# ashys2012/MDC-Net-Multimodal-Defect-Captioning-Network-For-Surface-Steel-Defects

Measured on NVIDIA B200. Metric: images/sec end-to-end encode+greedy decode, higher is better.
Workload: dtype bf16

## Files before the change

mdc-net-multimodal-defect-captioning-network-for-surface-steel-defects_b200/csrc/attention_umma.cu:

```cuda
#include "common.cuh"
#include <cuda.h>
#include <stdlib.h>

namespace {

constexpr int HD = 64;
constexpr int QROWS = 256;
constexpr int N_SOFTMAX_WARPS = 16;
constexpr int THREADS = 64 + N_SOFTMAX_WARPS * 32;

struct SmemLayout {
  int q_bytes, kv_bytes, buf_bytes;
};

__global__ void __launch_bounds__(THREADS, 1)
attn_umma_kernel(const __grid_constant__ CUtensorMap map_q, const __grid_constant__ CUtensorMap map_kv, bf16* __restrict__ out, int64_t ldo,
                 int n_items, int S, int H, int NK, float scale_log2e, long long* dbg) {
#ifdef MDC_DEVTOOLS
#define STAMP(i) do { if (dbg && blockIdx.x == 0 && n == 0) dbg[i] = clock64(); } while (0)
#else
#define STAMP(i) do { } while (0)
#endif
  extern __shared__ uint8_t smem_raw[];
  uint8_t* smem = (uint8_t*)(((uintptr_t)smem_raw + 1023) & ~(uintptr_t)1023);
  const int q_bytes = QROWS * 128, kv_bytes = NK * 128, buf_bytes = q_bytes + 2 * kv_bytes;
  uint64_t* bars = (uint64_t*)(smem + 2 * buf_bytes);
  uint64_t* full = bars; uint64_t* sfree = bars + 2; uint64_t* s_ready = bars + 4; uint64_t* p_ready = bars + 6; uint64_t* o_ready = bars + 8;
  uint64_t* t_free = bars + 10;
  uint32_t* tmem_ptr_smem = (uint32_t*)(bars + 12);
  float* xch = (float*)(bars + 16);
  const int warp = threadIdx.x >> 5, lane = threadIdx.x & 31;
  const int tiles = S > 128 ? 2 : 1;

  if (threadIdx.x == 0) {
    for (int i = 0; i < 2; ++i) {
      mbar_init(smem_u32(&full[i]), 1); mbar_init(smem_u32(&sfree[i]), 1); mbar_init(smem_u32(&s_ready[i]), 1);
      mbar_init(smem_u32(&p_ready[i]), N_SOFTMAX_WARPS * 32); mbar_init(smem_u32(&o_ready[i]), 1); mbar_init(smem_u32(&t_free[i]), N_SOFTMAX_WARPS * 32);
    }
    fence_mbarrier_init();
    prefetch_tmap(&map_q);
    prefetch_tmap(&map_kv);
  }
  if (warp == 0) {
    tmem_alloc<1>(smem_u32(tmem_ptr_smem), 512);
    tmem_relinquish<1>();
  }
  tc_fence_before();
  __syncthreads();
  tc_fence_after();
  const uint32_t tmem_base = *tmem_ptr_smem;
  const int D = H * HD;

  if (warp == 1) {
    if (lane == 0) {
      int n = 0;
      for (int item = blockIdx.x; item < n_items; item += gridDim.x, ++n) {
        const int buf = n & 1, strip = item / H, head = item % H;
        mbar_wait(smem_u32(&sfree[buf]), ((n >> 1) & 1) ^ 1);
        const uint32_t fb = smem_u32(&full[buf]);
        const uint32_t base = smem_u32(smem + buf * buf_bytes);
        STAMP(0);
        mbar_expect_tx(fb, (uint32_t)(3 * kv_bytes));
        tma_load_2d(&map_kv, fb, base, head * HD, strip * S);
        tma_load_2d(&map_kv, fb, base + q_bytes, D + head * HD, strip * S);
        tma_load_2d(&map_kv, fb, base + q_bytes + kv_bytes, 2 * D + head * HD, strip * S);
      }
    }
  } else if (warp == 0) {
    if (lane == 0) {
      const uint32_t idesc_qk = make_idesc(128, NK), idesc_pv = make_idesc(128, HD, false, true);
      int n = 0;
      for (int item = blockIdx.x; item < n_items; item += gridDim.x, ++n) {
        const int buf = n & 1;
        const uint32_t base = smem_u32(smem + buf * buf_bytes);
        mbar_wait(smem_u32(&full[buf]), (n >> 1) & 1);
        STAMP(1);
        tc_fence_after();
        const uint64_t kdesc = make_sw128_desc(base + q_bytes);
        for (int t = 0; t < tiles; ++t) {
          mbar_wait(smem_u32(&t_free[t]), (n & 1) ^ 1);
          tc_fence_after();
          const uint64_t qdesc = make_sw128_desc(base + t * 128 * 128);
#pragma unroll
          for (int k = 0; k < HD / 16; ++k) umma_ss(tmem_base + t * 256, qdesc + 2 * k, kdesc + 2 * k, idesc_qk, k != 0);
          umma_commit(smem_u32(&s_ready[t]));
          STAMP(2 + t);
        }
        const uint64_t vdesc = make_sw128_desc(base + q_bytes + kv_bytes);
        for (int t = 0; t < tiles; ++t) {
          mbar_wait(smem_u32(&p_ready[t]), n & 1);
          STAMP(4 + t);
          tc_fence_after();
          for (int k = 0; k < NK / 16; ++k)
            umma_ts(tmem_base + t * 256 + 128, tmem_base + t * 256 + 8 * k, vdesc + (uint64_t)(128 * k), idesc_pv, k != 0);
          umma_commit(smem_u32(&o_ready[t]));
          STAMP(6 + t);
        }
        umma_commit(smem_u32(&sfree[buf]));
      }
    }
  } else {
    const int sw = warp - 2, part = sw >> 2, row = 32 * (warp & 3) + lane;
    const int qc = NK / 4;
    const int nch = qc / 4;
    const uint32_t lane_addr = (uint32_t)(32 * (warp & 3)) << 16;
    int n = 0;
    for (int item = blockIdx.x; item < n_items; item += gridDim.x, ++n) {
      const int strip = item / H, head = item % H;
      float rsum[2] = {0.f, 0.f};
      for (int t = 0; t < tiles; ++t) {
        mbar_wait(smem_u32(&s_ready[t]), n & 1);
        if (threadIdx.x == 64) STAMP(10 + 8 * t);
        tc_fence_after();
        const uint32_t trow = tmem_base + lane_addr + t * 256;
        const bool live = __any_sync(0xffffffffu, t * 128 + row < S);
        float s[64];
        if (live) {
          uint32_t* sr = reinterpret_cast<uint32_t*>(s);
          const uint32_t tcol = trow + part * qc;
          if (nch >= 8) {
            tmem_ld32(tcol, sr);
            if (nch == 16) tmem_ld32(tcol + 32, sr + 32);
            else if (nch >= 12) {
              tmem_ld16(tcol + 32, sr + 32);
#pragma unroll
              for (int c = 12; c < 15; ++c) if (c < nch) tmem_ld4(tcol + 4 * c, sr + 4 * c);
            } else {
#pragma unroll
              for (int c = 8; c < 11; ++c) if (c < nch) tmem_ld4(tcol + 4 * c, sr + 4 * c);
            }
          } else if (nch >= 4) {
            tmem_ld16(tcol, sr);
#pragma unroll
            for (int c = 4; c < 7; ++c) if (c < nch) tmem_ld4(tcol + 4 * c, sr + 4 * c);
          } else {
#pragma unroll
            for (int c = 0; c < 3; ++c) if (c < nch) tmem_ld4(tcol + 4 * c, sr + 4 * c);
          }
          tmem_ld_wait();
        }
        if (threadIdx.x == 64) STAMP(11 + 8 * t);
        const int nvalid = min(max(S - part * qc, 0), qc);
        float m4[4] = {-INFINITY, -INFINITY, -INFINITY, -INFINITY};
        if (live) {
#pragma unroll
          for (int c = 0; c < 16; ++c)
            if (c < nch) {
              if (4 * c + 4 <= nvalid) {
#pragma unroll
                for (int j = 0; j < 4; ++j) m4[j] = fmaxf(m4[j], s[4 * c + j]);
              } else {
#pragma unroll
                for (int j = 0; j < 4; ++j) {
                  if (4 * c + j >= nvalid) s[4 * c + j] = -INFINITY;
                  m4[j] = fmaxf(m4[j], s[4 * c + j]);
                }
              }
            }
        }
        float mx = fmaxf(fmaxf(m4[0], m4[1]), fmaxf(m4[2], m4[3]));
        xch[part * 128 + row] = mx;
        bar_sync<128>(1 + (warp & 3));
        if (threadIdx.x == 64) STAMP(12 + 8 * t);
        mx = fmaxf(fmaxf(xch[row], xch[128 + row]), fmaxf(xch[256 + row], xch[384 + row]));
        const float nms = -mx * scale_log2e;
        float s4[4] = {0.f, 0.f, 0.f, 0.f};
        if (live) {
#pragma unroll
          for (int c = 0; c < 16; ++c)
            if (c < nch) {
              float p[4];
#pragma unroll
              for (int j = 0; j < 4; ++j) { p[j] = ex2_approx(fmaf(s[4 * c + j], scale_log2e, nms)); s4[j] += p[j]; }
              tmem_st2(trow + (part * qc) / 2 + 2 * c, pack_bf16x2(p[0], p[1]), pack_bf16x2(p[2], p[3]));
            }
        }
        const float sum = (s4[0] + s4[1]) + (s4[2] + s4[3]);
        rsum[t] = sum;
        xch[512 + t * 512 + part * 128 + row] = sum;
        if (threadIdx.x == 64) STAMP(13 + 8 * t);
        tmem_st_wait();
        if (threadIdx.x == 64) STAMP(14 + 8 * t);
        tc_fence_before();
        mbar_arrive(smem_u32(&p_ready[t]));
        bar_sync<128>(1 + (warp & 3));
      }
      for (int t = 0; t < tiles; ++t) {
        mbar_wait(smem_u32(&o_ready[t]), n & 1);
        if (threadIdx.x == 64) STAMP(26 + 2 * t);
        tc_fence_after();
        const uint32_t trow = tmem_base + lane_addr + t * 256 + 128;
        uint32_t o[16];
        tmem_ld16(trow + part * 16, o);
        tmem_ld_wait();
        tc_fence_before();
        mbar_arrive(smem_u32(&t_free[t]));
        const float* sx = xch + 512 + t * 512 + row;
        const float inv = 1.0f / ((sx[0] + sx[128]) + (sx[256] + sx[384]));
        const int q = t * 128 + row;
        if (q < S) {
          bf16* dst = out + ((int64_t)strip * S + q) * ldo + head * HD + part * 16;
#pragma unroll
          for (int j = 0; j < 16; j += 8) {
            uint4 v;
            v.x = pack_bf16x2(__uint_as_float(o[j]) * inv, __uint_as_float(o[j + 1]) * inv);
            v.y = pack_bf16x2(__uint_as_float(o[j + 2]) * inv, __uint_as_float(o[j + 3]) * inv);
            v.z = pack_bf16x2(__uint_as_float(o[j + 4]) * inv, __uint_as_float(o[j + 5]) * inv);
            v.w = pack_bf16x2(__uint_as_float(o[j + 6]) * inv, __uint_as_float(o[j + 7]) * inv);
            *reinterpret_cast<uint4*>(dst + j) = v;
          }
        }
      }
      if (threadIdx.x == 64) STAMP(30);
      bar_sync<128>(1 + (warp & 3));
    }
  }
  tc_fence_before();
  __syncthreads();
  if (warp == 0) {
    tc_fence_after();
    tmem_dealloc<1>(tmem_base, 512);
  }
}

}

int attn_umma_supported(int strip_len, int head_dim, int64_t ld, int64_t ldo) {
  return head_dim == HD && strip_len >= 16 && strip_len <= 256 && ld % 8 == 0 && ldo % 8 == 0;
}

int attn_umma_launch(mdc_ctx* ctx, const void* qkv, int64_t ld, void* out, int64_t ldo, int n_strips, int strip_len, int heads, float scale,
                     cudaStream_t s) {
  MDC_CHECK_ARG(((uintptr_t)qkv & 15) == 0 && ((uintptr_t)out & 15) == 0);
  const int S = strip_len, NK = ((S + 15) / 16) * 16;
  const int64_t rows = (int64_t)n_strips * S;
  CUtensorMap mq, mkv;
  MDC_TRY(mdc_make_tmap_2d(ctx, qkv, rows, 3 * heads * HD, ld, HD, NK, 3, &mkv));
  mq = mkv;
  const int buf_bytes = QROWS * 128 + 2 * NK * 128;
  const size_t smem = 2 * (size_t)buf_bytes + 1024 + 128 + 3 * 512 * 4;
  MDC_ENSURE_SMEM(attn_umma_kernel, smem);
  const int n_items = n_strips * heads;
  const int grid = n_items < ctx->sm_count ? n_items : ctx->sm_count;
  long long* dbg = nullptr;
#ifdef MDC_DEVTOOLS
  if (const char* e = getenv("MDC_ATTN_TRACE_PTR")) dbg = (long long*)strtoull(e, nullptr, 0);
#endif
  attn_umma_kernel<<<grid, THREADS, smem, s>>>(mq, mkv, (bf16*)out, ldo, n_items, S, heads, NK, scale * LOG2E, dbg);
  MDC_LAUNCH_CHECK(ctx);
  return 0;
}
```

mdc-net-multimodal-defect-captioning-network-for-surface-steel-defects_b200/csrc/ptx.cuh:

```cuda
#pragma once
#include <cuda.h>
#include <cuda_bf16.h>
#include <cuda_fp16.h>
#include <stdint.h>

__device__ __forceinline__ uint32_t smem_u32(const void* p) { return (uint32_t)__cvta_generic_to_shared(p); }
__device__ __forceinline__ uint32_t mapa(uint32_t addr, uint32_t rank) {
  uint32_t r; asm volatile("mapa.shared::cluster.u32 %0, %1, %2;" : "=r"(r) : "r"(addr), "r"(rank)); return r;
}
__device__ __forceinline__ uint32_t cluster_rank() { uint32_t r; asm volatile("mov.u32 %0, %%cluster_ctarank;" : "=r"(r)); return r; }
__device__ __forceinline__ void cluster_sync() {
  asm volatile("barrier.cluster.arrive.release.aligned;\n\tbarrier.cluster.wait.acquire.aligned;" ::: "memory");
}
__device__ __forceinline__ bool elect_one() {
  uint32_t pred;
  asm volatile("{\n\t.reg .pred P;\n\telect.sync _|P, 0xffffffff;\n\tselp.u32 %0, 1, 0, P;\n\t}\n" : "=r"(pred));
  return pred != 0;
}
__device__ __forceinline__ void st_async_b32(uint32_t raddr, uint32_t v, uint32_t rbar) {
  asm volatile("st.async.shared::cluster.mbarrier::complete_tx::bytes.b32 [%0], %1, [%2];" ::"r"(raddr), "r"(v), "r"(rbar) : "memory");
}

__device__ __forceinline__ void mbar_init(uint32_t bar, uint32_t count) {
  asm volatile("mbarrier.init.shared::cta.b64 [%0], %1;" ::"r"(bar), "r"(count) : "memory");
}
__device__ __forceinline__ void fence_mbarrier_init() { asm volatile("fence.mbarrier_init.release.cluster;" ::: "memory"); }
__device__ __forceinline__ void mbar_expect_tx(uint32_t bar, uint32_t bytes) {
  asm volatile("mbarrier.arrive.expect_tx.shared::cta.b64 _, [%0], %1;" ::"r"(bar), "r"(bytes) : "memory");
}
__device__ __forceinline__ void mbar_arrive(uint32_t bar) {
  asm volatile("mbarrier.arrive.shared::cta.b64 _, [%0];" ::"r"(bar) : "memory");
}
__device__ __forceinline__ void mbar_arrive_n(uint32_t bar, uint32_t count) {
  asm volatile("mbarrier.arrive.shared::cta.b64 _, [%0], %1;" ::"r"(bar), "r"(count) : "memory");
}
__device__ __forceinline__ void mbar_arrive_cluster(uint32_t local_bar, uint32_t cta) {
  const uint32_t r = mapa(local_bar, cta);
  asm volatile("mbarrier.arrive.shared::cluster.b64 _, [%0];" ::"r"(r) : "memory");
}
__device__ __forceinline__ void mbar_wait(uint32_t bar, uint32_t parity) {
  uint32_t done = 0, spins = 0;
  while (true) {
    asm volatile("{\n\t.reg .pred P1;\n\tmbarrier.try_wait.parity.shared::cta.b64 P1, [%1], %2, %3;\n\tselp.u32 %0, 1, 0, P1;\n\t}\n"
                 : "=r"(done) : "r"(bar), "r"(parity), "r"(1000000u) : "memory");
    if (done) break;
    if (++spins > 2000u) __trap();
  }
}
__device__ __forceinline__ void mbar_wait_spin(uint32_t bar, uint32_t parity) {
  uint32_t done = 0, spins = 0;
  long long t0 = 0;
  while (true) {
    asm volatile("{\n\t.reg .pred P1;\n\tmbarrier.try_wait.parity.shared::cta.b64 P1, [%1], %2;\n\tselp.u32 %0, 1, 0, P1;\n\t}\n"
                 : "=r"(done) : "r"(bar), "r"(parity) : "memory");
    if (done) break;
    if ((++spins & 1023u) == 0) {
      long long now = clock64();
      if (t0 == 0) t0 = now;
      else if (now - t0 > 4000000000LL) __trap();
    }
  }
}

__device__ __forceinline__ void cp_async16(uint32_t dst, const void* src) {
  asm volatile("cp.async.cg.shared.global [%0], [%1], 16;" ::"r"(dst), "l"(src) : "memory");
}
__device__ __forceinline__ void cp_async8(uint32_t dst, const void* src) {
  asm volatile("cp.async.ca.shared.global [%0], [%1], 8;" ::"r"(dst), "l"(src) : "memory");
}
__device__ __forceinline__ void cp_async_commit() { asm volatile("cp.async.commit_group;" ::: "memory"); }
template <int N> __device__ __forceinline__ void cp_async_wait() { asm volatile("cp.async.wait_group %0;" ::"n"(N) : "memory"); }
__device__ __forceinline__ void cp_async_wait_all() { cp_async_commit(); cp_async_wait<0>(); }
__device__ __forceinline__ void prefetch_l2(const void* p) { asm volatile("prefetch.global.L2 [%0];" ::"l"(p)); }
__device__ __forceinline__ void bulk_g2s(uint32_t dst, const void* src, uint32_t bytes, uint32_t bar) {
  asm volatile("cp.async.bulk.shared::cluster.global.mbarrier::complete_tx::bytes [%0], [%1], %2, [%3];"
               ::"r"(dst), "l"(src), "r"(bytes), "r"(bar) : "memory");
}
__device__ __forceinline__ void bulk_prefetch_l2(const void* src, uint32_t bytes) {
  asm volatile("cp.async.bulk.prefetch.L2.global [%0], %1;" ::"l"(src), "r"(bytes) : "memory");
}
__device__ __forceinline__ void prefetch_tmap(const CUtensorMap* map) { asm volatile("prefetch.tensormap [%0];" ::"l"(map) : "memory"); }
__device__ __forceinline__ void tma_load_2d(const CUtensorMap* map, uint32_t bar, uint32_t dst, int c0, int c1) {
  asm volatile("cp.async.bulk.tensor.2d.shared::cluster.global.mbarrier::complete_tx::bytes [%0], [%1, {%3, %4}], [%2];"
               ::"r"(dst), "l"(map), "r"(bar), "r"(c0), "r"(c1) : "memory");
}
__device__ __forceinline__ void tma_load_2d_2sm(const CUtensorMap* map, uint32_t leader_bar, uint32_t dst, int c0, int c1) {
  asm volatile("cp.async.bulk.tensor.2d.cta_group::2.shared::cluster.global.mbarrier::complete_tx::bytes [%0], [%1, {%3, %4}], [%2];"
               ::"r"(dst), "l"(map), "r"(leader_bar), "r"(c0), "r"(c1) : "memory");
}
__device__ __forceinline__ void tma_store_2d(const CUtensorMap* map, uint32_t src, int c0, int c1) {
  asm volatile("cp.async.bulk.tensor.2d.global.shared::cta.bulk_group [%0, {%2, %3}], [%1];" ::"l"(map), "r"(src), "r"(c0), "r"(c1) : "memory");
}
__device__ __forceinline__ void tma_reduce_add_2d(const CUtensorMap* map, uint32_t src, int c0, int c1) {
  asm volatile("cp.reduce.async.bulk.tensor.2d.global.shared::cta.add.tile.bulk_group [%0, {%2, %3}], [%1];" ::"l"(map), "r"(src), "r"(c0), "r"(c1) : "memory");
}
__device__ __forceinline__ void bulk_commit() { asm volatile("cp.async.bulk.commit_group;" ::: "memory"); }
template <int N> __device__ __forceinline__ void bulk_wait_read() { asm volatile("cp.async.bulk.wait_group.read %0;" ::"n"(N) : "memory"); }
__device__ __forceinline__ void fence_proxy_async() { asm volatile("fence.proxy.async;" ::: "memory"); }
__device__ __forceinline__ void fence_proxy_async_smem() { asm volatile("fence.proxy.async.shared::cta;" ::: "memory"); }

__device__ __forceinline__ void ldsm_x4(uint32_t* r, uint32_t addr) {
  asm volatile("ldmatrix.sync.aligned.m8n8.x4.shared.b16 {%0,%1,%2,%3}, [%4];" : "=r"(r[0]), "=r"(r[1]), "=r"(r[2]), "=r"(r[3]) : "r"(addr));
}
__device__ __forceinline__ void ldsm_x4_trans(uint32_t* r, uint32_t addr) {
  asm volatile("ldmatrix.sync.aligned.m8n8.x4.trans.shared.b16 {%0,%1,%2,%3}, [%4];" : "=r"(r[0]), "=r"(r[1]), "=r"(r[2]), "=r"(r[3]) : "r"(addr));
}
template <int HD>
__device__ __forceinline__ uint32_t swz(int r, int c) {
  if constexpr (HD == 32) return (uint32_t)(r * 64 + ((c ^ ((r >> 1) & 3)) << 4));
  else return (uint32_t)(r * (HD * 2) + ((c ^ (r & 7)) << 4));
}
template <typename T> __device__ __forceinline__ void mma_m16n8k16(float* c, const uint32_t* a, uint32_t b0, uint32_t b1);
template <> __device__ __forceinline__ void mma_m16n8k16<__nv_bfloat16>(float* c, const uint32_t* a, uint32_t b0, uint32_t b1) {
  asm volatile("mma.sync.aligned.m16n8k16.row.col.f32.bf16.bf16.f32 {%0,%1,%2,%3}, {%4,%5,%6,%7}, {%8,%9}, {%0,%1,%2,%3};"
               : "+f"(c[0]), "+f"(c[1]), "+f"(c[2]), "+f"(c[3]) : "r"(a[0]), "r"(a[1]), "r"(a[2]), "r"(a[3]), "r"(b0), "r"(b1));
}
template <> __device__ __forceinline__ void mma_m16n8k16<__half>(float* c, const uint32_t* a, uint32_t b0, uint32_t b1) {
  asm volatile("mma.sync.aligned.m16n8k16.row.col.f32.f16.f16.f32 {%0,%1,%2,%3}, {%4,%5,%6,%7}, {%8,%9}, {%0,%1,%2,%3};"
               : "+f"(c[0]), "+f"(c[1]), "+f"(c[2]), "+f"(c[3]) : "r"(a[0]), "r"(a[1]), "r"(a[2]), "r"(a[3]), "r"(b0), "r"(b1));
}

__device__ __forceinline__ void tc_fence_before() { asm volatile("tcgen05.fence::before_thread_sync;" ::: "memory"); }
__device__ __forceinline__ void tc_fence_after() { asm volatile("tcgen05.fence::after_thread_sync;" ::: "memory"); }
__device__ __forceinline__ void umma_ss(uint32_t tmem_d, uint64_t adesc, uint64_t bdesc, uint32_t idesc, uint32_t accumulate) {
  asm volatile("{\n\t.reg .pred p;\n\tsetp.ne.b32 p, %4, 0;\n\ttcgen05.mma.cta_group::1.kind::f16 [%0], %1, %2, %3, p;\n\t}\n"
               ::"r"(tmem_d), "l"(adesc), "l"(bdesc), "r"(idesc), "r"(accumulate) : "memory");
}
__device__ __forceinline__ void umma_ts(uint32_t tmem_d, uint32_t tmem_a, uint64_t bdesc, uint32_t idesc, uint32_t accumulate) {
  asm volatile("{\n\t.reg .pred p;\n\tsetp.ne.b32 p, %4, 0;\n\ttcgen05.mma.cta_group::1.kind::f16 [%0], [%1], %2, %3, p;\n\t}\n"
               ::"r"(tmem_d), "r"(tmem_a), "l"(bdesc), "r"(idesc), "r"(accumulate) : "memory");
}
__device__ __forceinline__ void umma_ss_2sm(uint32_t tmem_d, uint64_t adesc, uint64_t bdesc, uint32_t idesc, uint32_t accumulate) {
  asm volatile("{\n\t.reg .pred p;\n\tsetp.ne.b32 p, %4, 0;\n\ttcgen05.mma.cta_group::2.kind::f16 [%0], %1, %2, %3, p;\n\t}\n"
               ::"r"(tmem_d), "l"(adesc), "l"(bdesc), "r"(idesc), "r"(accumulate) : "memory");
}
__device__ __forceinline__ void umma_commit(uint32_t bar) {
  asm volatile("tcgen05.commit.cta_group::1.mbarrier::arrive::one.shared::cluster.b64 [%0];" ::"r"(bar) : "memory");
}
__device__ __forceinline__ void umma_commit_2sm(uint32_t bar) {
  asm volatile("tcgen05.commit.cta_group::2.mbarrier::arrive::one.shared::cluster.multicast::cluster.b64 [%0], %1;" ::"r"(bar), "h"((uint16_t)3) : "memory");
}
__device__ __forceinline__ void tmem_ld4(uint32_t addr, uint32_t* v) {
  asm volatile("tcgen05.ld.sync.aligned.32x32b.x4.b32 {%0, %1, %2, %3}, [%4];" : "=r"(v[0]), "=r"(v[1]), "=r"(v[2]), "=r"(v[3]) : "r"(addr));
}
__device__ __forceinline__ void tmem_ld16(uint32_t addr, uint32_t* v) {
  asm volatile("tcgen05.ld.sync.aligned.32x32b.x16.b32 {%0, %1, %2, %3, %4, %5, %6, %7, %8, %9, %10, %11, %12, %13, %14, %15}, [%16];"
               : "=r"(v[0]), "=r"(v[1]), "=r"(v[2]), "=r"(v[3]), "=r"(v[4]), "=r"(v[5]), "=r"(v[6]), "=r"(v[7]),
                 "=r"(v[8]), "=r"(v[9]), "=r"(v[10]), "=r"(v[11]), "=r"(v[12]), "=r"(v[13]), "=r"(v[14]), "=r"(v[15]) : "r"(addr));
}
__device__ __forceinline__ void tmem_ld32(uint32_t addr, uint32_t* v) {
  asm volatile("tcgen05.ld.sync.aligned.32x32b.x32.b32 "
               "{%0, %1, %2, %3, %4, %5, %6, %7, %8, %9, %10, %11, %12, %13, %14, %15, "
               "%16, %17, %18, %19, %20, %21, %22, %23, %24, %25, %26, %27, %28, %29, %30, %31}, [%32];"
               : "=r"(v[0]), "=r"(v[1]), "=r"(v[2]), "=r"(v[3]), "=r"(v[4]), "=r"(v[5]), "=r"(v[6]), "=r"(v[7]),
                 "=r"(v[8]), "=r"(v[9]), "=r"(v[10]), "=r"(v[11]), "=r"(v[12]), "=r"(v[13]), "=r"(v[14]), "=r"(v[15]),
                 "=r"(v[16]), "=r"(v[17]), "=r"(v[18]), "=r"(v[19]), "=r"(v[20]), "=r"(v[21]), "=r"(v[22]), "=r"(v[23]),
                 "=r"(v[24]), "=r"(v[25]), "=r"(v[26]), "=r"(v[27]), "=r"(v[28]), "=r"(v[29]), "=r"(v[30]), "=r"(v[31])
               : "r"(addr));
}
__device__ __forceinline__ void tmem_ld_wait() { asm volatile("tcgen05.wait::ld.sync.aligned;" ::: "memory"); }
__device__ __forceinline__ void tmem_st2(uint32_t addr, uint32_t a, uint32_t b) {
  asm volatile("tcgen05.st.sync.aligned.32x32b.x2.b32 [%0], {%1, %2};" ::"r"(addr), "r"(a), "r"(b) : "memory");
}
__device__ __forceinline__ void tmem_st_wait() { asm volatile("tcgen05.wait::st.sync.aligned;" ::: "memory"); }
template <int CG> __device__ __forceinline__ void tmem_alloc(uint32_t dst, uint32_t cols) {
  if constexpr (CG == 2) asm volatile("tcgen05.alloc.cta_group::2.sync.aligned.shared::cta.b32 [%0], %1;" ::"r"(dst), "r"(cols) : "memory");
  else asm volatile("tcgen05.alloc.cta_group::1.sync.aligned.shared::cta.b32 [%0], %1;" ::"r"(dst), "r"(cols) : "memory");
}
template <int CG> __device__ __forceinline__ void tmem_relinquish() {
  if constexpr (CG == 2) asm volatile("tcgen05.relinquish_alloc_permit.cta_group::2.sync.aligned;" ::: "memory");
  else asm volatile("tcgen05.relinquish_alloc_permit.cta_group::1.sync.aligned;" ::: "memory");
}
template <int CG> __device__ __forceinline__ void tmem_dealloc(uint32_t base, uint32_t cols) {
  if constexpr (CG == 2) asm volatile("tcgen05.dealloc.cta_group::2.sync.aligned.b32 %0, %1;" ::"r"(base), "r"(cols) : "memory");
  else asm volatile("tcgen05.dealloc.cta_group::1.sync.aligned.b32 %0, %1;" ::"r"(base), "r"(cols) : "memory");
}
__device__ __forceinline__ uint64_t make_sw128_desc(uint32_t saddr) {
  uint64_t d = 0;
  d |= (uint64_t)((saddr >> 4) & 0x3FFF);
  d |= (uint64_t)(1024 >> 4) << 32;
  d |= (uint64_t)1 << 46;
  d |= (uint64_t)2 << 61;
  return d;
}
__host__ __device__ constexpr uint32_t make_idesc(int M, int N, bool f16 = false, bool b_mn_major = false) {
  return (1u << 4) | ((f16 ? 0u : 1u) << 7) | ((f16 ? 0u : 1u) << 10) | ((b_mn_major ? 1u : 0u) << 16) | ((uint32_t)(N >> 3) << 17) |
         ((uint32_t)(M >> 4) << 24);
}

__device__ __forceinline__ uint4 lds128(uint32_t addr) {
  uint4 v; asm volatile("ld.shared.v4.u32 {%0,%1,%2,%3}, [%4];" : "=r"(v.x), "=r"(v.y), "=r"(v.z), "=r"(v.w) : "r"(addr)); return v;
}
__device__ __forceinline__ void sts128(uint32_t addr, uint32_t a, uint32_t b, uint32_t c, uint32_t d) {
  asm volatile("st.shared.v4.b32 [%0], {%1, %2, %3, %4};" ::"r"(addr), "r"(a), "r"(b), "r"(c), "r"(d) : "memory");
}
template <int ID, int COUNT> __device__ __forceinline__ void bar_sync() { asm volatile("bar.sync %0, %1;" ::"n"(ID), "n"(COUNT) : "memory"); }
template <int COUNT> __device__ __forceinline__ void bar_sync(uint32_t id) { asm volatile("bar.sync %0, %1;" ::"r"(id), "n"(COUNT) : "memory"); }

__device__ __forceinline__ float ex2_approx(float x) { float y; asm("ex2.approx.ftz.f32 %0, %1;" : "=f"(y) : "f"(x)); return y; }
__device__ __forceinline__ uint64_t pk2(float a, float b) { uint64_t r; asm("mov.b64 %0, {%1, %2};" : "=l"(r) : "f"(a), "f"(b)); return r; }
__device__ __forceinline__ void upk2(uint64_t v, float& a, float& b) { asm("mov.b64 {%0, %1}, %2;" : "=f"(a), "=f"(b) : "l"(v)); }
__device__ __forceinline__ uint64_t fma2(uint64_t a, uint64_t b, uint64_t c) { uint64_t d; asm("fma.rn.f32x2 %0, %1, %2, %3;" : "=l"(d) : "l"(a), "l"(b), "l"(c)); return d; }
__device__ __forceinline__ uint64_t add2(uint64_t a, uint64_t b) { uint64_t d; asm("add.rn.f32x2 %0, %1, %2;" : "=l"(d) : "l"(a), "l"(b)); return d; }

__device__ __forceinline__ uint32_t pack_bf16x2(float a, float b) { __nv_bfloat162 h = __floats2bfloat162_rn(a, b); return *reinterpret_cast<uint32_t*>(&h); }
__device__ __forceinline__ uint32_t pack_f16x2(float a, float b) { __half2 h = __floats2half2_rn(a, b); return *reinterpret_cast<uint32_t*>(&h); }
```

Measured before the change: 13190.

## Split attention into per-tile work units and overlap QK, softmax and epilogue across units

```diff
diff --git a/mdc-net-multimodal-defect-captioning-network-for-surface-steel-defects_b200/csrc/attention_umma.cu b/mdc-net-multimodal-defect-captioning-network-for-surface-steel-defects_b200/csrc/attention_umma.cu
--- a/mdc-net-multimodal-defect-captioning-network-for-surface-steel-defects_b200/csrc/attention_umma.cu
+++ b/mdc-net-multimodal-defect-captioning-network-for-surface-steel-defects_b200/csrc/attention_umma.cu
@@ -5,19 +5,15 @@
 namespace {
 
 constexpr int HD = 64;
-constexpr int QROWS = 256;
+constexpr int QROWS = 128;
 constexpr int N_SOFTMAX_WARPS = 16;
 constexpr int THREADS = 64 + N_SOFTMAX_WARPS * 32;
 
-struct SmemLayout {
-  int q_bytes, kv_bytes, buf_bytes;
-};
-
 __global__ void __launch_bounds__(THREADS, 1)
 attn_umma_kernel(const __grid_constant__ CUtensorMap map_q, const __grid_constant__ CUtensorMap map_kv, bf16* __restrict__ out, int64_t ldo,
-                 int n_items, int S, int H, int NK, float scale_log2e, long long* dbg) {
+                 int n_units, int tiles, int S, int H, int NK, float scale_log2e, long long* dbg) {
 #ifdef MDC_DEVTOOLS
-#define STAMP(i) do { if (dbg && blockIdx.x == 0 && n == 0) dbg[i] = clock64(); } while (0)
+#define STAMP(i) do { if (dbg && blockIdx.x == 0 && n >= 4 && n < 6) dbg[32 * (n - 4) + (i)] = clock64(); } while (0)
 #else
 #define STAMP(i) do { } while (0)
 #endif
@@ -30,7 +26,6 @@
   uint32_t* tmem_ptr_smem = (uint32_t*)(bars + 12);
   float* xch = (float*)(bars + 16);
   const int warp = threadIdx.x >> 5, lane = threadIdx.x & 31;
-  const int tiles = S > 128 ? 2 : 1;
 
   if (threadIdx.x == 0) {
     for (int i = 0; i < 2; ++i) {
@@ -54,14 +49,14 @@
   if (warp == 1) {
     if (lane == 0) {
       int n = 0;
-      for (int item = blockIdx.x; item < n_items; item += gridDim.x, ++n) {
-        const int buf = n & 1, strip = item / H, head = item % H;
+      for (int u = blockIdx.x; u < n_units; u += gridDim.x, ++n) {
+        const int buf = n & 1, item = u / tiles, t = u - item * tiles, strip = item / H, head = item % H;
         mbar_wait(smem_u32(&sfree[buf]), ((n >> 1) & 1) ^ 1);
         const uint32_t fb = smem_u32(&full[buf]);
         const uint32_t base = smem_u32(smem + buf * buf_bytes);
         STAMP(0);
-        mbar_expect_tx(fb, (uint32_t)(3 * kv_bytes));
-        tma_load_2d(&map_kv, fb, base, head * HD, strip * S);
+        mbar_expect_tx(fb, (uint32_t)(q_bytes + 2 * kv_bytes));
+        tma_load_2d(&map_q, fb, base, head * HD, strip * S + t * QROWS);
         tma_load_2d(&map_kv, fb, base + q_bytes, D + head * HD, strip * S);
         tma_load_2d(&map_kv, fb, base + q_bytes + kv_bytes, 2 * D + head * HD, strip * S);
       }
@@ -69,151 +64,148 @@
   } else if (warp == 0) {
     if (lane == 0) {
       const uint32_t idesc_qk = make_idesc(128, NK), idesc_pv = make_idesc(128, HD, false, true);
+      auto issue_qk = [&](int n) {
+        const int r = n & 1;
+        const uint32_t base = smem_u32(smem + r * buf_bytes);
+        mbar_wait(smem_u32(&full[r]), (n >> 1) & 1);
+        STAMP(1);
+        mbar_wait(smem_u32(&t_free[r]), ((n >> 1) & 1) ^ 1);
+        tc_fence_after();
+        const uint64_t qdesc = make_sw128_desc(base), kdesc = make_sw128_desc(base + q_bytes);
+#pragma unroll
+        for (int k = 0; k < HD / 16; ++k) umma_ss(tmem_base + r * 256, qdesc + 2 * k, kdesc + 2 * k, idesc_qk, k != 0);
+        umma_commit(smem_u32(&s_ready[r]));
+        STAMP(2);
+      };
       int n = 0;
-      for (int item = blockIdx.x; item < n_items; item += gridDim.x, ++n) {
-        const int buf = n & 1;
-        const uint32_t base = smem_u32(smem + buf * buf_bytes);
-        mbar_wait(smem_u32(&full[buf]), (n >> 1) & 1);
-        STAMP(1);
+      issue_qk(0);
+      for (int u = blockIdx.x; u < n_units; u += gridDim.x, ++n) {
+        if (u + (int)gridDim.x < n_units) issue_qk(n + 1);
+        const int r = n & 1;
+        mbar_wait(smem_u32(&p_ready[r]), (n >> 1) & 1);
+        STAMP(3);
         tc_fence_after();
-        const uint64_t kdesc = make_sw128_desc(base + q_bytes);
-        for (int t = 0; t < tiles; ++t) {
-          mbar_wait(smem_u32(&t_free[t]), (n & 1) ^ 1);
-          tc_fence_after();
-          const uint64_t qdesc = make_sw128_desc(base + t * 128 * 128);
-#pragma unroll
-          for (int k = 0; k < HD / 16; ++k) umma_ss(tmem_base + t * 256, qdesc + 2 * k, kdesc + 2 * k, idesc_qk, k != 0);
-          umma_commit(smem_u32(&s_ready[t]));
-          STAMP(2 + t);
-        }
-        const uint64_t vdesc = make_sw128_desc(base + q_bytes + kv_bytes);
-        for (int t = 0; t < tiles; ++t) {
-          mbar_wait(smem_u32(&p_ready[t]), n & 1);
-          STAMP(4 + t);
-          tc_fence_after();
-          for (int k = 0; k < NK / 16; ++k)
-            umma_ts(tmem_base + t * 256 + 128, tmem_base + t * 256 + 8 * k, vdesc + (uint64_t)(128 * k), idesc_pv, k != 0);
-          umma_commit(smem_u32(&o_ready[t]));
-          STAMP(6 + t);
-        }
-        umma_commit(smem_u32(&sfree[buf]));
+        const uint64_t vdesc = make_sw128_desc(smem_u32(smem + r * buf_bytes) + q_bytes + kv_bytes);
+        for (int k = 0; k < NK / 16; ++k)
+          umma_ts(tmem_base + r * 256 + 128, tmem_base + r * 256 + 8 * k, vdesc + (uint64_t)(128 * k), idesc_pv, k != 0);
+        umma_commit(smem_u32(&o_ready[r]));
+        umma_commit(smem_u32(&sfree[r]));
+        STAMP(4);
       }
     }
   } else {
     const int sw = warp - 2, part = sw >> 2, row = 32 * (warp & 3) + lane;
     const int qc = NK / 4;
     const int nch = qc / 4;
+    const int nvalid = min(max(S - part * qc, 0), qc);
     const uint32_t lane_addr = (uint32_t)(32 * (warp & 3)) << 16;
-    int n = 0;
-    for (int item = blockIdx.x; item < n_items; item += gridDim.x, ++n) {
-      const int strip = item / H, head = item % H;
-      float rsum[2] = {0.f, 0.f};
-      for (int t = 0; t < tiles; ++t) {
-        mbar_wait(smem_u32(&s_ready[t]), n & 1);
-        if (threadIdx.x == 64) STAMP(10 + 8 * t);
-        tc_fence_after();
-        const uint32_t trow = tmem_base + lane_addr + t * 256;
-        const bool live = __any_sync(0xffffffffu, t * 128 + row < S);
-        float s[64];
-        if (live) {
-          uint32_t* sr = reinterpret_cast<uint32_t*>(s);
-          const uint32_t tcol = trow + part * qc;
-          if (nch >= 8) {
-            tmem_ld32(tcol, sr);
-            if (nch == 16) tmem_ld32(tcol + 32, sr + 32);
-            else if (nch >= 12) {
-              tmem_ld16(tcol + 32, sr + 32);
-#pragma unroll
-              for (int c = 12; c < 15; ++c) if (c < nch) tmem_ld4(tcol + 4 * c, sr + 4 * c);
+    auto epilogue = [&](int n, int item, int t) {
+      const int r = n & 1;
+      mbar_wait(smem_u32(&o_ready[r]), (n >> 1) & 1);
+      tc_fence_after();
+      uint32_t o[16];
+      tmem_ld16(tmem_base + lane_addr + r * 256 + 128 + part * 16, o);
+      tmem_ld_wait();
+      tc_fence_before();
+      mbar_arrive(smem_u32(&t_free[r]));
+      const float* sx = xch + 512 + r * 512 + row;
+      const float inv = 1.0f / ((sx[0] + sx[128]) + (sx[256] + sx[384]));
+      const int q = t * QROWS + row;
+      if (q < S) {
+        bf16* dst = out + ((int64_t)(item / H) * S + q) * ldo + (item % H) * HD + part * 16;
+#pragma unroll
+        for (int j = 0; j < 16; j += 8) {
+          uint4 v;
+          v.x = pack_bf16x2(__uint_as_float(o[j]) * inv, __uint_as_float(o[j + 1]) * inv);
+          v.y = pack_bf16x2(__uint_as_float(o[j + 2]) * inv, __uint_as_float(o[j + 3]) * inv);
+          v.z = pack_bf16x2(__uint_as_float(o[j + 4]) * inv, __uint_as_float(o[j + 5]) * inv);
+          v.w = pack_bf16x2(__uint_as_float(o[j + 6]) * inv, __uint_as_float(o[j + 7]) * inv);
+          *reinterpret_cast<uint4*>(dst + j) = v;
+        }
+      }
+    };
+    int n = 0, prev_item = 0, prev_t = 0;
+    for (int u = blockIdx.x; u < n_units; u += gridDim.x, ++n) {
+      const int r = n & 1, item = u / tiles, t = u - item * tiles;
+      mbar_wait(smem_u32(&s_ready[r]), (n >> 1) & 1);
+      if (threadIdx.x == 64) STAMP(10);
+      tc_fence_after();
+      const uint32_t trow = tmem_base + lane_addr + r * 256;
+      const bool live = __any_sync(0xffffffffu, t * QROWS + row < S);
+      float s[64];
+      if (live) {
+        uint32_t* sr = reinterpret_cast<uint32_t*>(s);
+        const uint32_t tcol = trow + part * qc;
+        if (nch >= 8) {
+          tmem_ld32(tcol, sr);
+          if (nch == 16) tmem_ld32(tcol + 32, sr + 32);
+          else if (nch >= 12) {
+            tmem_ld16(tcol + 32, sr + 32);
+#pragma unroll
+            for (int c = 12; c < 15; ++c) if (c < nch) tmem_ld4(tcol + 4 * c, sr + 4 * c);
+          } else {
+#pragma unroll
+            for (int c = 8; c < 11; ++c) if (c < nch) tmem_ld4(tcol + 4 * c, sr + 4 * c);
+          }
+        } else if (nch >= 4) {
+          tmem_ld16(tcol, sr);
+#pragma unroll
+          for (int c = 4; c < 7; ++c) if (c < nch) tmem_ld4(tcol + 4 * c, sr + 4 * c);
+        } else {
+#pragma unroll
+          for (int c = 0; c < 3; ++c) if (c < nch) tmem_ld4(tcol + 4 * c, sr + 4 * c);
+        }
+      }
+      tmem_ld_wait();
+      if (threadIdx.x == 64) STAMP(12);
+      float m4[4] = {-INFINITY, -INFINITY, -INFINITY, -INFINITY};
+      if (live) {
+#pragma unroll
+        for (int c = 0; c < 16; ++c)
+          if (c < nch) {
+            if (4 * c + 4 <= nvalid) {
+#pragma unroll
+              for (int j = 0; j < 4; ++j) m4[j] = fmaxf(m4[j], s[4 * c + j]);
             } else {
 #pragma unroll
-              for (int c = 8; c < 11; ++c) if (c < nch) tmem_ld4(tcol + 4 * c, sr + 4 * c);
-            }
-          } else if (nch >= 4) {
-            tmem_ld16(tcol, sr);
-#pragma unroll
-            for (int c = 4; c < 7; ++c) if (c < nch) tmem_ld4(tcol + 4 * c, sr + 4 * c);
-          } else {
-#pragma unroll
-            for (int c = 0; c < 3; ++c) if (c < nch) tmem_ld4(tcol + 4 * c, sr + 4 * c);
-          }
-          tmem_ld_wait();
-        }
-        if (threadIdx.x == 64) STAMP(11 + 8 * t);
-        const int nvalid = min(max(S - part * qc, 0), qc);
-        float m4[4] = {-INFINITY, -INFINITY, -INFINITY, -INFINITY};
-        if (live) {
-#pragma unroll
-          for (int c = 0; c < 16; ++c)
-            if (c < nch) {
-              if (4 * c + 4 <= nvalid) {
-#pragma unroll
-                for (int j = 0; j < 4; ++j) m4[j] = fmaxf(m4[j], s[4 * c + j]);
-              } else {
-#pragma unroll
-                for (int j = 0; j < 4; ++j) {
-                  if (4 * c + j >= nvalid) s[4 * c + j] = -INFINITY;
-                  m4[j] = fmaxf(m4[j], s[4 * c + j]);
-                }
+              for (int j = 0; j < 4; ++j) {
+                if (4 * c + j >= nvalid) s[4 * c + j] = -INFINITY;
+                m4[j] = fmaxf(m4[j], s[4 * c + j]);
               }
             }
-        }
-        float mx = fmaxf(fmaxf(m4[0], m4[1]), fmaxf(m4[2], m4[3]));
-        xch[part * 128 + row] = mx;
-        bar_sync<128>(1 + (warp & 3));
-        if (threadIdx.x == 64) STAMP(12 + 8 * t);
-        mx = fmaxf(fmaxf(xch[row], xch[128 + row]), fmaxf(xch[256 + row], xch[384 + row]));
-        const float nms = -mx * scale_log2e;
-        float s4[4] = {0.f, 0.f, 0.f, 0.f};
-        if (live) {
-#pragma unroll
-          for (int c = 0; c < 16; ++c)
-            if (c < nch) {
-              float p[4];
+          }
+      }
+      float mx = fmaxf(fmaxf(m4[0], m4[1]), fmaxf(m4[2], m4[3]));
+      xch[part * 128 + row] = mx;
+      bar_sync<128>(1 + (warp & 3));
+      if (threadIdx.x == 64) STAMP(13);
+      mx = fmaxf(fmaxf(xch[row], xch[128 + row]), fmaxf(xch[256 + row], xch[384 + row]));
+      const float nms = -mx * scale_log2e;
+      float s4[4] = {0.f, 0.f, 0.f, 0.f};
+      if (live) {
+#pragma unroll
+        for (int c = 0; c < 16; ++c)
+          if (c < nch) {
+            float p[4] = {0.f, 0.f, 0.f, 0.f};
+            if (4 * c < nvalid) {
 #pragma unroll
               for (int j = 0; j < 4; ++j) { p[j] = ex2_approx(fmaf(s[4 * c + j], scale_log2e, nms)); s4[j] += p[j]; }
-              tmem_st2(trow + (part * qc) / 2 + 2 * c, pack_bf16x2(p[0], p[1]), pack_bf16x2(p[2], p[3]));
             }
-        }
-        const float sum = (s4[0] + s4[1]) + (s4[2] + s4[3]);
-        rsum[t] = sum;
-        xch[512 + t * 512 + part * 128 + row] = sum;
-        if (threadIdx.x == 64) STAMP(13 + 8 * t);
-        tmem_st_wait();
-        if (threadIdx.x == 64) STAMP(14 + 8 * t);
-        tc_fence_before();
-        mbar_arrive(smem_u32(&p_ready[t]));
-        bar_sync<128>(1 + (warp & 3));
-      }
-      for (int t = 0; t < tiles; ++t) {
-        mbar_wait(smem_u32(&o_ready[t]), n & 1);
-        if (threadIdx.x == 64) STAMP(26 + 2 * t);
-        tc_fence_after();
-        const uint32_t trow = tmem_base + lane_addr + t * 256 + 128;
-        uint32_t o[16];
-        tmem_ld16(trow + part * 16, o);
-        tmem_ld_wait();
-        tc_fence_before();
-        mbar_arrive(smem_u32(&t_free[t]));
-        const float* sx = xch + 512 + t * 512 + row;
-        const float inv = 1.0f / ((sx[0] + sx[128]) + (sx[256] + sx[384]));
-        const int q = t * 128 + row;
-        if (q < S) {
-          bf16* dst = out + ((int64_t)strip * S + q) * ldo + head * HD + part * 16;
-#pragma unroll
-          for (int j = 0; j < 16; j += 8) {
-            uint4 v;
-            v.x = pack_bf16x2(__uint_as_float(o[j]) * inv, __uint_as_float(o[j + 1]) * inv);
-            v.y = pack_bf16x2(__uint_as_float(o[j + 2]) * inv, __uint_as_float(o[j + 3]) * inv);
-            v.z = pack_bf16x2(__uint_as_float(o[j + 4]) * inv, __uint_as_float(o[j + 5]) * inv);
-            v.w = pack_bf16x2(__uint_as_float(o[j + 6]) * inv, __uint_as_float(o[j + 7]) * inv);
-            *reinterpret_cast<uint4*>(dst + j) = v;
+            tmem_st2(trow + (part * qc) / 2 + 2 * c, pack_bf16x2_alu(p[0], p[1]), pack_bf16x2_alu(p[2], p[3]));
           }
-        }
-      }
-      if (threadIdx.x == 64) STAMP(30);
+      }
+      xch[512 + r * 512 + part * 128 + row] = (s4[0] + s4[1]) + (s4[2] + s4[3]);
+      if (threadIdx.x == 64) STAMP(14);
+      tmem_st_wait();
+      if (threadIdx.x == 64) STAMP(15);
+      tc_fence_before();
+      mbar_arrive(smem_u32(&p_ready[r]));
+      if (n > 0) epilogue(n - 1, prev_item, prev_t);
+      if (threadIdx.x == 64) STAMP(11);
       bar_sync<128>(1 + (warp & 3));
-    }
+      prev_item = item; prev_t = t;
+    }
+    if (n > 0) epilogue(n - 1, prev_item, prev_t);
   }
   tc_fence_before();
   __syncthreads();
@@ -232,21 +224,21 @@
 int attn_umma_launch(mdc_ctx* ctx, const void* qkv, int64_t ld, void* out, int64_t ldo, int n_strips, int strip_len, int heads, float scale,
                      cudaStream_t s) {
   MDC_CHECK_ARG(((uintptr_t)qkv & 15) == 0 && ((uintptr_t)out & 15) == 0);
-  const int S = strip_len, NK = ((S + 15) / 16) * 16;
+  const int S = strip_len, NK = ((S + 15) / 16) * 16, tiles = S > QROWS ? 2 : 1;
   const int64_t rows = (int64_t)n_strips * S;
   CUtensorMap mq, mkv;
+  MDC_TRY(mdc_make_tmap_2d(ctx, qkv, rows, 3 * heads * HD, ld, HD, QROWS, 3, &mq));
   MDC_TRY(mdc_make_tmap_2d(ctx, qkv, rows, 3 * heads * HD, ld, HD, NK, 3, &mkv));
-  mq = mkv;
   const int buf_bytes = QROWS * 128 + 2 * NK * 128;
   const size_t smem = 2 * (size_t)buf_bytes + 1024 + 128 + 3 * 512 * 4;
   MDC_ENSURE_SMEM(attn_umma_kernel, smem);
-  const int n_items = n_strips * heads;
-  const int grid = n_items < ctx->sm_count ? n_items : ctx->sm_count;
+  const int n_units = n_strips * heads * tiles;
+  const int grid = n_units < ctx->sm_count ? n_units : ctx->sm_count;
   long long* dbg = nullptr;
 #ifdef MDC_DEVTOOLS
   if (const char* e = getenv("MDC_ATTN_TRACE_PTR")) dbg = (long long*)strtoull(e, nullptr, 0);
 #endif
-  attn_umma_kernel<<<grid, THREADS, smem, s>>>(mq, mkv, (bf16*)out, ldo, n_items, S, heads, NK, scale * LOG2E, dbg);
+  attn_umma_kernel<<<grid, THREADS, smem, s>>>(mq, mkv, (bf16*)out, ldo, n_units, tiles, S, heads, NK, scale * LOG2E, dbg);
   MDC_LAUNCH_CHECK(ctx);
   return 0;
 }
diff --git a/mdc-net-multimodal-defect-captioning-network-for-surface-steel-defects_b200/csrc/ptx.cuh b/mdc-net-multimodal-defect-captioning-network-for-surface-steel-defects_b200/csrc/ptx.cuh
--- a/mdc-net-multimodal-defect-captioning-network-for-surface-steel-defects_b200/csrc/ptx.cuh
+++ b/mdc-net-multimodal-defect-captioning-network-for-surface-steel-defects_b200/csrc/ptx.cuh
@@ -204,4 +204,8 @@
 __device__ __forceinline__ uint64_t add2(uint64_t a, uint64_t b) { uint64_t d; asm("add.rn.f32x2 %0, %1, %2;" : "=l"(d) : "l"(a), "l"(b)); return d; }
 
 __device__ __forceinline__ uint32_t pack_bf16x2(float a, float b) { __nv_bfloat162 h = __floats2bfloat162_rn(a, b); return *reinterpret_cast<uint32_t*>(&h); }
+__device__ __forceinline__ uint32_t pack_bf16x2_alu(float a, float b) {
+  const uint32_t ua = __float_as_uint(a), ub = __float_as_uint(b);
+  return __byte_perm(ua + 0x7fffu + ((ua >> 16) & 1u), ub + 0x7fffu + ((ub >> 16) & 1u), 0x7632);
+}
 __device__ __forceinline__ uint32_t pack_f16x2(float a, float b) { __half2 h = __floats2half2_rn(a, b); return *reinterpret_cast<uint32_t*>(&h); }
```

Measured after the change: 13140 (median of 6 runs). No clear change (-0.3%).
